# eps696/aphantasia

Hardware: AMD Instinct MI355X
Metric: optimization steps/sec @1280x720 ViT-B/32 samples=200 (higher is better)
Workload: dtype f16 (MFMA operands, fp32 accumulate; fp32 residual stream / LayerNorm / softmax statistics / synth / sampler / loss / Adam)

## Files before the change

### aphantasia_amd/_ffi.py

```python
import ctypes
import os
from ctypes import POINTER, c_char_p, c_float, c_int, c_size_t, c_void_p

import torch

HERE = os.path.dirname(os.path.abspath(__file__))
LIB_PATH = os.path.join(HERE, 'libaphantasia_hip.so')

APH_OUT_NCHW_RAW, APH_OUT_NCHW_NORM, APH_OUT_PATCH_F16, APH_GRAD_PATCH_F16, APH_OUT_PATCH_F16_HILO, APH_OUT_PATCH_F32 = 0, 1, 2, 3, 4, 5
APH_AUG_STRIDE = 16
SIM_TYPES = {'cossim': 0, 'cos': 0, None: 0, 'mix': 1, 'ang': 2, 'dot': 3}


class SampleGeom(ctypes.Structure):
    _fields_ = [(n, c_int) for n in ('H', 'W', 'Hp', 'Wp', 'py0', 'px0', 'S', 'size', 'patch')]


_PROTOTYPES = {
    'aph_version': (c_int, []),
    'aph_last_error': (c_char_p, []),
    'aph_synth_plan_create': (c_int, [c_int, c_int, c_int, POINTER(c_void_p)]),
    'aph_synth_plan_destroy': (c_int, [c_void_p]),
    'aph_synth_fft_fwd': (c_int, [c_void_p, c_void_p, c_void_p, c_void_p, c_float, POINTER(c_float), c_int, c_void_p, c_void_p, c_void_p]),
    'aph_synth_fft_bwd': (c_int, [c_void_p, c_void_p, c_float, c_void_p, c_void_p, c_void_p, c_float, POINTER(c_float), c_int, c_void_p, c_void_p]),
    'aph_irfft2': (c_int, [c_void_p, c_void_p, c_void_p, c_void_p]),
    'aph_rfft2': (c_int, [c_void_p, c_void_p, c_void_p, c_void_p]),
    'aph_synth_spatial_fwd': (c_int, [c_void_p, c_void_p, c_float, c_float, POINTER(c_float), c_int, c_void_p, c_void_p]),
    'aph_synth_spatial_bwd': (c_int, [c_void_p, c_void_p, c_float, c_void_p, c_void_p, c_float, c_float, POINTER(c_float), c_int, c_void_p, c_void_p]),
    'aph_synth_stats': (c_int, [c_void_p, c_void_p, c_void_p]),
    'aph_synth_set_stats': (c_int, [c_void_p, c_void_p, c_void_p]),
    'aph_synth_plan_describe': (c_int, [c_void_p, POINTER(c_int)]),
    'aph_idwt_coarse_levels': (c_int, [POINTER(c_int), POINTER(c_int), c_int, c_int]),
    'aph_rgb_priors_ws_bytes': (c_size_t, []),
    'aph_rgb_sharp': (c_int, [c_void_p, c_int, c_int, c_float, c_void_p, c_void_p, c_void_p, c_void_p]),
    'aph_rgb_priors': (c_int, [c_void_p, c_int, c_int, c_float, c_float, c_float, c_void_p, c_void_p, c_void_p, c_void_p]),
    'aph_cppn_param_count': (c_size_t, [c_int, c_int, c_int]),
    'aph_cppn_ws_bytes': (c_size_t, [c_int, c_int, c_int, c_int, c_int]),
    'aph_cppn_fwd': (c_int, [c_void_p, c_int, c_int, c_int, c_void_p, c_void_p, c_int, c_int, c_void_p, c_void_p, c_void_p]),
    'aph_cppn_bwd': (c_int, [c_void_p, c_int, c_int, c_int, c_void_p, c_void_p, c_int, c_int, c_void_p, c_float, c_void_p, c_void_p, c_void_p, c_void_p]),
    'aph_idwt_level_fwd': (c_int, [c_void_p, c_int, c_int, c_void_p, c_int, c_int, c_int, c_void_p, c_void_p, c_int, c_float, c_void_p, c_void_p]),
    'aph_idwt_fwd': (c_int, [c_void_p, c_void_p, c_void_p, c_void_p, c_void_p, c_int, c_int, c_void_p, c_void_p, c_int, c_void_p, c_void_p]),
    'aph_idwt_bwd': (c_int, [c_void_p, c_void_p, c_void_p, c_void_p, c_int, c_int, c_void_p, c_void_p, c_int, c_void_p, c_void_p, c_void_p, c_void_p]),
    'aph_idwt_level_bwd': (c_int, [c_void_p, c_int, c_int, c_int, c_void_p, c_void_p, c_int, c_float, c_void_p, c_int, c_int, c_void_p, c_void_p]),
    'aph_sample_ws_bytes': (c_size_t, [POINTER(SampleGeom), c_int]),
    'aph_sample_fwd': (c_int, [POINTER(SampleGeom), c_void_p, c_void_p, c_void_p, c_void_p, c_void_p, c_int, c_void_p]),
    'aph_sample_bwd': (c_int, [POINTER(SampleGeom), c_void_p, c_float, c_void_p, c_void_p, c_void_p, c_void_p, c_int, c_void_p]),
    'aph_triangle_blur': (c_int, [c_void_p, c_int, c_int, c_int, c_int, c_float, c_float, c_void_p, c_void_p]),
    'aph_resize_bicubic': (c_int, [c_void_p, c_int, c_int, c_int, c_void_p, c_int, c_int, c_void_p]),
    'aph_flip_w': (c_int, [c_void_p, c_void_p, c_int, c_int, c_int, c_void_p, c_void_p]),
    'aph_grid_warp': (c_int, [c_void_p, c_void_p, c_int, c_int, c_int, c_float, c_float, c_float, c_float, c_float, c_void_p, c_void_p, c_void_p]),
    'aph_attn_test': (c_int, [c_void_p, c_void_p, c_void_p, c_void_p, c_void_p, c_void_p, c_int, c_int, c_int, c_int, c_void_p]),
    'aph_attn_f32_test': (c_int, [c_void_p, c_void_p, c_void_p, c_void_p, c_void_p, c_void_p, c_int, c_int, c_int, c_int, c_void_p]),
    'aph_frame_affine': (c_int, [c_void_p, c_int, c_int, c_int, POINTER(c_float), c_void_p, c_void_p]),
    'aph_patchify_f16': (c_int, [c_void_p, c_int, c_int, c_int, c_void_p, c_void_p]),
    'aph_patchify_f16_hilo': (c_int, [c_void_p, c_int, c_int, c_int, c_void_p, c_void_p]),
    'aph_patchify_f32': (c_int, [c_void_p, c_int, c_int, c_int, c_void_p, c_void_p]),
    'aph_unpatchify_f32': (c_int, [c_void_p, c_int, c_int, c_int, c_float, c_void_p, c_void_p]),
    'aph_vit_create': (c_int, [c_int, c_int, c_int, c_int, c_int, c_int, c_int, POINTER(c_void_p)]),
    'aph_vit_destroy': (c_int, [c_void_p]),
    'aph_vit_workspace_bytes': (c_size_t, [c_void_p]),
    'aph_vit_set_weight': (c_int, [c_void_p, c_char_p, c_void_p, c_size_t]),
    'aph_vit_forward': (c_int, [c_void_p, c_void_p, c_int, c_void_p, c_void_p]),
    'aph_vit_forward_hilo': (c_int, [c_void_p, c_void_p, c_int, c_void_p, c_void_p]),
    'aph_vit_enable_hilo': (c_int, [c_void_p]),
    'aph_vit_enable_f32': (c_int, [c_void_p]),
    'aph_vit_forward_f32': (c_int, [c_void_p, c_void_p, c_int, c_void_p, c_void_p]),
    'aph_vit_backward_f32': (c_int, [c_void_p, c_void_p, c_int, c_void_p, c_float, c_void_p]),
    'aph_vit_backward': (c_int, [c_void_p, c_void_p, c_int, c_void_p, c_float, c_void_p]),
    'aph_vit_backward_h': (c_int, [c_void_p, c_void_p, c_int, c_void_p, c_float, c_void_p]),
    'aph_vit_profile': (c_int, [c_void_p, c_int]),
    'aph_vit_profile_read': (c_int, [c_void_p, c_void_p, c_void_p, c_void_p]),
    'aph_gemm_set_mfma32': (c_int, [c_int]),
    'aph_vit_set_fuse_ln': (c_int, [c_int]),
    'aph_crop_adjoint_set_gather': (c_int, [c_int]),
    'aph_crop_adjoint_set_shape': (c_int, [c_int, c_int, c_int, c_int, c_int]),
    'aph_vit_set_grad_stream_f16': (c_int, [c_int]),
    'aph_gemm_set_ws_min_tiles': (c_int, [c_int]),
    'aph_gemm_set_ws_pgroup': (c_int, [c_int]),
    'aph_gemm_set_rs': (c_int, [c_int]),
    'aph_mfma_rate': (c_int, [c_int, c_int, c_void_p, c_void_p, c_void_p]),
    'aph_gemm_rs_probe': (c_int, [c_void_p, c_void_p, c_int, c_int, c_int, c_void_p, c_int, c_void_p, c_void_p]),
    'aph_gemm_ws_probe': (c_int, [c_void_p, c_void_p, c_int, c_int, c_int, c_void_p, c_void_p, c_void_p, c_int, c_void_p, c_void_p]),
    'aph_gemm_f32_test': (c_int, [c_void_p, c_int, c_int, c_void_p, c_int, c_int, c_int, c_int, c_void_p, c_int, c_void_p, c_void_p, c_int, c_void_p, c_size_t, c_void_p]),
    'aph_gemm_f16': (c_int, [c_void_p, c_void_p, c_int, c_int, c_int, c_void_p, c_void_p]),
    'aph_gemm_f16_ld': (c_int, [c_void_p, c_int, c_void_p, c_int, c_int, c_int, c_int, c_void_p, c_int, c_void_p]),
    'aph_gemm_f16_epi_test': (c_int, [c_void_p, c_int, c_void_p, c_int, c_int, c_int, c_int, c_void_p, c_int, c_void_p, c_void_p, c_void_p, c_float, c_int,
                                      c_int, c_int, c_int, c_void_p, c_size_t, c_int, c_void_p]),
    'aph_ln_test': (c_int, [c_int, c_int, c_int, c_int, c_int, c_int, c_int, c_void_p, c_void_p, c_void_p, c_void_p, c_void_p, c_void_p, c_void_p,
                            c_void_p, c_void_p, c_void_p, c_void_p, c_void_p, c_void_p, c_void_p]),
    'aph_sim_loss': (c_int, [c_void_p, c_int, c_int, c_void_p, c_void_p, POINTER(c_float), c_int, c_int, c_int, c_int, c_int, c_float, c_float, c_void_p, c_void_p, c_void_p, c_void_p]),
    'aph_axpy_f32': (c_int, [c_void_p, c_void_p, c_float, c_size_t, c_void_p]),
    'aph_rgb_to_u8': (c_int, [c_void_p, c_int, c_int, c_float, c_void_p, c_void_p]),
    'aph_linear_head': (c_int, [c_void_p, c_int, c_int, c_void_p, c_float, c_float, c_float, c_float, c_void_p, c_void_p, c_void_p]),
    'aph_comm_unique_id': (c_int, [c_void_p]),
    'aph_comm_init': (c_int, [c_int, c_int, c_void_p, POINTER(c_void_p)]),
    'aph_allreduce_f32': (c_int, [c_void_p, c_void_p, c_size_t, c_void_p]),
    'aph_comm_ranks': (c_int, [c_void_p, POINTER(c_int)]),
    'aph_comm_destroy': (c_int, [c_void_p]),
    'aph_adam_step': (c_int, [c_void_p, c_void_p, c_void_p, c_void_p, c_void_p, c_void_p, c_int, c_size_t, c_void_p]),
    'aph_adam_step_guarded': (c_int, [c_void_p, c_void_p, c_void_p, c_void_p, c_void_p, c_void_p, c_int, c_size_t, c_void_p, c_void_p]),
}

EXPORTS = tuple(_PROTOTYPES)

class Library:

    def __init__(self, path):
        if not os.path.isfile(path):
            raise RuntimeError(
                "aphantasia_amd: HIP library not found at %s -- build it with "
                "`python -c 'import __graft_entry__ as g; g.build()'` (hipcc, gfx950). "
                "There is no CPU fallback." % path)
        self.path = path
        self.cdll = ctypes.CDLL(path)
        for name, (res, args) in _PROTOTYPES.items():
            fn = getattr(self.cdll, name)
            fn.restype = res
            fn.argtypes = args

    def last_error(self):
        return (self.cdll.aph_last_error() or b'').decode(errors='replace')

    def call(self, name, *args):
        rc = getattr(self.cdll, name)(*args)
        if rc < 0:
            raise RuntimeError('%s failed (%d): %s' % (name, rc, self.last_error()))
        return rc


_lib = None


def lib():
    global _lib
    if _lib is None:
        import torch
        if torch.cuda.is_available():
            torch.cuda.init()
            torch.empty(1, device='cuda')
        _lib = Library(LIB_PATH)
    return _lib


def ptr(t):
    return c_void_p(t.data_ptr()) if t is not None else c_void_p(0)


def floats(seq):
    if seq is None:
        return None
    arr = (c_float * len(seq))(*[float(v) for v in seq])
    return arr
```

### aphantasia_amd/csrc/vit_gemm_ws.h

```cpp
#pragma once
#include "vit_gemm.h"

namespace aph {

template <int BM_, int NPROD_, int NSTAGE_, int WG_PER_CU_, int BIAS_MAX_, int FORCE_WAVES_ = 0>
struct GemmWSCfg {
  static constexpr int BM = BM_, BN = 128, WM = BM / 64, WN = 2, NCONS = WM * WN, NPROD = NPROD_, NWAVE = NCONS + NPROD, NTHREAD = NWAVE * 64;
  static constexpr int NSTAGE = NSTAGE_, WG_PER_CU = WG_PER_CU_;
  static constexpr int STAGE = (BM + BN) * GEMM_BK;
  static constexpr int SMEM = NSTAGE * STAGE * 2;
  static constexpr int BIAS_MAX = BIAS_MAX_;
  static constexpr int SMEM_TOTAL = SMEM + BIAS_MAX * 4;
  static constexpr int QA = BM / 8, QB = BN / 8;
  static constexpr int QPW = (QA + QB) / NPROD;
  static constexpr int QAW = QA / NPROD;
  static constexpr int MIN_WAVES_PER_SIMD = FORCE_WAVES_ ? FORCE_WAVES_ : (WG_PER_CU * NWAVE + 3) / 4;
  static_assert(QA % NPROD == 0 && QB % NPROD == 0 && (NSTAGE - 1) * QPW <= 63, "the DMA in flight must fit the vmcnt range");
  static_assert(WG_PER_CU * SMEM_TOTAL <= 160 * 1024 && NSTAGE >= 2 && NSTAGE <= 3, "LDS budget / ring depth");
};
using GemmWS = GemmWSCfg<256, 2, 3, 1, 4096>;

__host__ __device__ __forceinline__ int gemm_ws_brow(int v) {
  const int vv = v & 63, nt = vv >> 4, i = vv & 15;
  return (v & ~63) + (i << 2) + nt;
}

__device__ __forceinline__ half4 pack_h4(float a, float b, float c, float d) { return half4{(half_t)a, (half_t)b, (half_t)c, (half_t)d}; }

#define APH_WS_ROWS(r, m4, M) for (int r = 0; r < 4; ++r) if ((m4) + r < (M))
__device__ __forceinline__ void ws_tile(const EpiF16& e, int m4, int M, int n4, f32x4 (&v)[4], const float* lb) {
  f32x4 b = {0.f, 0.f, 0.f, 0.f};
  if (e.bias) b = *reinterpret_cast<const f32x4*>(lb + n4);
#pragma unroll
  APH_WS_ROWS(r, m4, M)
    *reinterpret_cast<half4*>(e.out + (size_t)(m4 + r) * e.ldo + n4) = pack_h4(v[0][r] + b[0], v[1][r] + b[1], v[2][r] + b[2], v[3][r] + b[3]);
}
__device__ __forceinline__ void ws_tile(const EpiF16Scale& e, int m4, int M, int n4, f32x4 (&v)[4], const float*) {
#pragma unroll
  APH_WS_ROWS(r, m4, M)
    *reinterpret_cast<half4*>(e.out + (size_t)(m4 + r) * e.ldo + n4) = pack_h4(v[0][r] * e.scale, v[1][r] * e.scale, v[2][r] * e.scale, v[3][r] * e.scale);
}
__device__ __forceinline__ void ws_tile(const EpiF32& e, int m4, int M, int n4, f32x4 (&v)[4], const float*) {
#pragma unroll
  APH_WS_ROWS(r, m4, M) st4(e.out + (size_t)(m4 + r) * e.ldo + n4, f32x4{v[0][r], v[1][r], v[2][r], v[3][r]} * e.scale);
}
__device__ __forceinline__ void ws_tile(const EpiNoStore& e, int m4, int M, int n4, f32x4 (&v)[4], const float*) {
  const f32x4 t = v[0] + v[1] + v[2] + v[3];
  if (m4 < M && t[0] + t[1] + t[2] + t[3] == 1.2345678e33f) st4(e.out + (size_t)m4 * e.ldo + n4, t);
}
__device__ __forceinline__ void ws_tile(const EpiResidual& e, int m4, int M, int n4, f32x4 (&v)[4], const float*) {
#pragma unroll
  APH_WS_ROWS(r, m4, M) st4(e.out + (size_t)(m4 + r) * e.ldo + n4, f32x4{v[0][r], v[1][r], v[2][r], v[3][r]});
}
__device__ __forceinline__ void ws_tile(const EpiPatchEmbed& e, int m4, int M, int n4, f32x4 (&v)[4], const float*) {
#pragma unroll
  APH_WS_ROWS(r, m4, M) {
    const int m = m4 + r, s = m / e.P, p = m - s * e.P;
    st4(e.x0 + ((size_t)s * e.T + 1 + p) * e.D + n4, f32x4{v[0][r], v[1][r], v[2][r], v[3][r]} + ld4(e.pos + (size_t)(1 + p) * e.D + n4));
  }
}
__device__ __forceinline__ void ws_tile(const EpiGelu& e, int m4, int M, int n4, f32x4 (&v)[4], const float* lb) {
  const f32x4 b = *reinterpret_cast<const f32x4*>(lb + n4);
#pragma unroll
  for (int r = 0; r < 4; ++r) {
    f32x4 gl, dg;
    quick_gelu4(f32x4{v[0][r] + b[0], v[1][r] + b[1], v[2][r] + b[2], v[3][r] + b[3]}, gl, dg);
    if (m4 + r < M) {
      *reinterpret_cast<half4*>(e.g + (size_t)(m4 + r) * e.ldo + n4) = pack_h4(gl[0], gl[1], gl[2], gl[3]);
      *reinterpret_cast<half4*>(e.dg + (size_t)(m4 + r) * e.ldo + n4) = pack_h4(dg[0], dg[1], dg[2], dg[3]);
    }
  }
}
__device__ __forceinline__ void ws_tile(const EpiGeluBwd& e, int m4, int M, int n4, f32x4 (&v)[4], const half4 (&d)[4]) {
#pragma unroll
  APH_WS_ROWS(r, m4, M)
    *reinterpret_cast<half4*>(e.out + (size_t)(m4 + r) * e.ldo + n4) =
        pack_h4(v[0][r] * (float)d[r][0], v[1][r] * (float)d[r][1], v[2][r] * (float)d[r][2], v[3][r] * (float)d[r][3]);
}
#undef APH_WS_ROWS
template <class E>
__device__ __forceinline__ void ws_tiles(const E& e, int m4, int M, int n4, f32x4 (&acc)[4][4], const float* lb) {
#pragma unroll
  for (int mt = 0; mt < 4; ++mt) ws_tile(e, m4 + mt * 16, M, n4, acc[mt], lb);
}
__device__ __forceinline__ void ws_tiles(const EpiGeluBwd& e, int m4, int M, int n4, f32x4 (&acc)[4][4], const float*) {
  half4 d[4][4];
#pragma unroll
  for (int mt = 0; mt < 4; ++mt)
#pragma unroll
    for (int r = 0; r < 4; ++r) {
      const int m = m4 + mt * 16 + r;
      d[mt][r] = *reinterpret_cast<const half4*>(e.dg + (size_t)(m < M ? m : M - 1) * e.ldo + n4);
    }
#pragma unroll
  for (int mt = 0; mt < 4; ++mt) ws_tile(e, m4 + mt * 16, M, n4, acc[mt], d[mt]);
}
template <class E>
__device__ __forceinline__ void ws_init(const E&, int, int, int, f32x4 (&v)[4], const float*) {
#pragma unroll
  for (int j = 0; j < 4; ++j) v[j] = f32x4{0.f, 0.f, 0.f, 0.f};
}
__device__ __forceinline__ void ws_init(const EpiResidual& e, int m4, int M, int n4, f32x4 (&v)[4], const float*) {
  const f32x4 b = ld4(e.bias + n4);
#pragma unroll
  for (int r = 0; r < 4; ++r) {
    const int m = m4 + r < M ? m4 + r : M - 1;
    const f32x4 x = ld4(e.res + (size_t)m * e.ldo + n4) + b;
    v[0][r] = x[0]; v[1][r] = x[1]; v[2][r] = x[2]; v[3][r] = x[3];
  }
}
__device__ __forceinline__ const float* ws_bias(const EpiF16& e) { return e.bias; }
__device__ __forceinline__ const float* ws_bias(const EpiResidual& e) { return e.bias; }
__device__ __forceinline__ const float* ws_bias(const EpiGelu& e) { return e.bias; }
template <class E> __device__ __forceinline__ const float* ws_bias(const E&) { return nullptr; }

__device__ __forceinline__ unsigned long long ws_realtime() {
#ifdef APH_EMU
  return 0ull;
#else
  return __builtin_amdgcn_s_memrealtime();
#endif
}
__device__ __forceinline__ unsigned long long ws_clock() {
#ifdef APH_EMU
  return 0ull;
#else
  return __builtin_amdgcn_s_memtime();
#endif
}

template <int AHEAD_UNIT>
__device__ __forceinline__ void ws_wait_barrier(int ahead) {
  if (ahead <= 0) wait_vm_barrier<0>();
  else if (ahead == 1) wait_vm_barrier<AHEAD_UNIT>();
  else wait_vm_barrier<(2 * AHEAD_UNIT <= 63 ? 2 * AHEAD_UNIT : 63)>();
}

template <class C, class Epi>
__global__ __launch_bounds__(C::NTHREAD, C::MIN_WAVES_PER_SIMD) void gemm_ws_kernel(const half_t* __restrict__ A, int lda, const half_t* __restrict__ Bt,
                                                                  int ldb, int M, int N, int K, Epi epi, int ntiles, int pgroup, unsigned long long* __restrict__ trace,
                                                                  int ntn_short, int nk_short) {
  using F = GemmBig;
  APH_DYN_SMEM(smem);
  half_t* lds = reinterpret_cast<half_t*>(smem);
  const int tid = threadIdx.x, lane = tid & 63, wave = wave_uniform(tid >> 6);
  const int nk = K / GEMM_BK, ntn = N / C::BN, ntm = ntiles / ntn, ntn_long = ntn - ntn_short;
  int pos, pos_end, tile_step, lstart, sstart, nlong;
  {
    const int nwg = gridDim.x, b = blockIdx.x, G = nwg < 8 ? nwg : 8, xcd = b % G;
    auto share = [&](int n, int& start, int& count) {
      const int q = n / G, r = n - q * G;
      start = xcd < r ? xcd * (q + 1) : r * (q + 1) + (xcd - r) * q;
      count = q + (xcd < r ? 1 : 0);
    };
    int nshort;
    share(ntm * ntn_long, lstart, nlong);
    share(ntm * ntn_short, sstart, nshort);
    pos_end = nlong + nshort;
    tile_step = (nwg - xcd + G - 1) / G;
    pos = b / G;
  }
  if (pos >= pos_end) return;
  if (trace && tid == 0) trace[((size_t)blockIdx.x * 16 + 15) * 4 + 3] = ws_realtime();
  int U = 0;
  for (int q = pos; q < pos_end; q += tile_step) U += q < nlong ? nk : nk_short;
  auto coords = [&](int q, int& tm, int& tn) -> int {
    const bool lng = q < nlong;
    const int t = lng ? lstart + q : sstart + (q - nlong), cols = lng ? ntn_long : ntn_short;
    const int per = pgroup * cols, g = t / per, rem = t - g * per;
    const int left = ntm - g * pgroup, rg = left < pgroup ? left : pgroup;
    tn = rem / rg;
    tm = g * pgroup + (rem - tn * rg);
    if (!lng) tn += ntn_long;
    return lng ? nk : nk_short;
  };
  float* lbias = reinterpret_cast<float*>(smem + C::SMEM);
  if (const float* gb = ws_bias(epi)) {
    for (int i = tid * 4; i < N; i += C::NTHREAD * 4) *reinterpret_cast<f32x4*>(lbias + i) = ld4(gb + i);
    wait_lgkm0();
  }

  if (wave >= C::NCONS) {
    const int p = wave - C::NCONS, lrow = lane >> 3, pc = lane & 7;
    unsigned off[C::QPW];
    const char* Ab = reinterpret_cast<const char*>(A);
    const char* Bb = reinterpret_cast<const char*>(Bt);
    int nk_it = nk;
    auto setup = [&](int t) {
      int tm, tn;
      nk_it = coords(t, tm, tn);
      const int n0 = tn * C::BN, m0 = tm * C::BM;
#pragma unroll
      for (int i = 0; i < C::QPW; ++i) {
        if (i < C::QAW) {
          const int row = (i * C::NPROD + p) * 8 + lrow;
          int am = m0 + row; am = am < M ? am : M - 1;
          off[i] = ((unsigned)am * (unsigned)lda + ((pc ^ ((row >> 1) & 7)) << 3)) * 2u;
        } else {
          const int v = ((i - C::QAW) * C::NPROD + p) * 8 + lrow;
          off[i] = ((unsigned)(n0 + gemm_ws_brow(v)) * (unsigned)ldb + ((pc ^ ((v >> 1) & 7)) << 3)) * 2u;
        }
      }
    };
    auto issue = [&](int kt, int stage) {
      half_t* As = lds + stage * C::STAGE;
      half_t* Bs = As + C::BM * GEMM_BK;
      const char* ak = Ab + (size_t)kt * (GEMM_BK * 2);
      const char* bk = Bb + (size_t)kt * (GEMM_BK * 2);
#pragma unroll
      for (int i = 0; i < C::QPW; ++i) {
        if (i < C::QAW) glds16(ak + off[i], As + (i * C::NPROD + p) * 8 * GEMM_BK);
        else glds16(bk + off[i], Bs + ((i - C::QAW) * C::NPROD + p) * 8 * GEMM_BK);
      }
    };
    int it = pos, ikt = 0, ist = 0, issued = 0;
    setup(it);
    auto issue_next = [&]() {
      issue(ikt, ist);
      ist = ist == C::NSTAGE - 1 ? 0 : ist + 1;
      ++issued;
      if (++ikt == nk_it) {
        ikt = 0;
        it += tile_step;
        if (issued < U) setup(it);
      }
    };
    const int pre = U < C::NSTAGE - 1 ? U : C::NSTAGE - 1;
    for (int i = 0; i < pre; ++i) issue_next();
    ws_wait_barrier<C::QPW>(pre - 1);
    if (U > C::NSTAGE - 1) issue_next();
    for (int u = 0; u + 1 < U; ++u) {
      const int rem = U - u - 2;
      ws_wait_barrier<C::QPW>(rem < C::NSTAGE - 2 ? rem : C::NSTAGE - 2);
      if (u + C::NSTAGE < U) issue_next();
    }
    return;
  }

  const int wm = wave / C::WN, wn = wave - wm * C::WN;
  f32x4 acc[F::TM][F::TN];
  const int frow = lane & 15, arow = wm * 64 + frow, brow = wn * 64 + frow, fchunk = lane >> 4;
  GemmFrags<F> f0, f1;
  int kt = 0, st = 0, nk_c = nk, ti = 0;
  auto init_tile = [&](int t) {
    int tm, tn;
    nk_c = coords(t, tm, tn);
    const int m4 = tm * C::BM + wm * 64 + 4 * (lane >> 4), n4 = tn * C::BN + wn * 64 + 4 * (lane & 15);
#pragma unroll
    for (int mt = 0; mt < F::TM; ++mt) ws_init(epi, m4 + mt * 16, M, n4, acc[mt], lbias);
  };
  auto mma = [&](const GemmFrags<F>& f) {
#pragma unroll
    for (int mt = 0; mt < F::TM; ++mt)
#pragma unroll
      for (int nt = 0; nt < F::TN; ++nt) acc[mt][nt] = mfma_16x16x32_f16(f.a[mt], f.b[nt], acc[mt][nt]);
  };
  init_tile(pos);
  wait_vm_barrier<63>();
  gemm_load_frags<F>(f0, lds, lds + C::BM * GEMM_BK, arow, brow, fchunk);
  for (int u = 0; u < U; ++u) {
    const half_t* As = lds + st * C::STAGE;
    st = st == C::NSTAGE - 1 ? 0 : st + 1;
    gemm_load_frags<F>(f1, As, As + C::BM * GEMM_BK, arow, brow, 4 + fchunk);
    mma(f0);
    if (u + 1 < U) {
      wait_lgkm0();
      wait_vm_barrier<63>();
      const half_t* An = lds + st * C::STAGE;
      gemm_load_frags<F>(f0, An, An + C::BM * GEMM_BK, arow, brow, fchunk);
    }
    mma(f1);
    if (trace && kt == 0 && tid == 0 && ti < 14) trace[((size_t)blockIdx.x * 16 + ti) * 4 + 0] = ws_clock();
    if (++kt == nk_c) {
      if (trace && tid == 0 && ti < 14) trace[((size_t)blockIdx.x * 16 + ti) * 4 + 1] = ws_clock();
      int tm, tn;
      coords(pos, tm, tn);
      const int m4 = tm * C::BM + wm * 64 + 4 * (lane >> 4), n4 = tn * C::BN + wn * 64 + 4 * (lane & 15);
      ws_tiles(epi, m4, M, n4, acc, lbias);
      if (trace && tid == 0 && ti < 14) trace[((size_t)blockIdx.x * 16 + ti) * 4 + 2] = ws_clock();
      kt = 0;
      ++ti;
      pos += tile_step;
      if (u + 1 < U) init_tile(pos);
    }
  }
  if (trace && tid == 0) trace[((size_t)blockIdx.x * 16 + 14) * 4 + 3] = ws_realtime();
}

inline int& gemm_ws_pgroup_override() {
  static int v = 0;
  return v;
}
inline int gemm_ws_panel_group(int ntn, int ntm) {
  int g = gemm_ws_pgroup_override();
  if (g <= 0) g = ntn >= 12 ? 4 : 1;
  return g < ntm ? g : (ntm > 0 ? ntm : 1);
}

template <class C, class Epi>
inline void launch_gemm_ws_cfg(const half_t* A, int lda, const half_t* Bt, int ldb, int M, int N, int K, Epi epi, hipStream_t st,
                               unsigned long long* trace, int n_short = 0, int k_short = 0) {
  const int ntiles = (N / C::BN) * ((M + C::BM - 1) / C::BM);
  const int cus = gemm_persistent_wgs();
  const int wgs = cus > (1 << 20) ? cus : cus * C::WG_PER_CU;
  APH_ALLOW_SMEM((gemm_ws_kernel<C, Epi>), C::SMEM_TOTAL);
  APH_LAUNCH((gemm_ws_kernel<C, Epi>), dim3(ntiles < wgs ? ntiles : wgs), dim3(C::NTHREAD), C::SMEM_TOTAL, st, A, lda, Bt, ldb, M, N, K, epi, ntiles,
             gemm_ws_panel_group(N / C::BN, (M + C::BM - 1) / C::BM), trace, n_short / C::BN, k_short / GEMM_BK);
}
template <class Epi>
inline void launch_gemm_ws(const half_t* A, int lda, const half_t* Bt, int ldb, int M, int N, int K, Epi epi, hipStream_t st,
                           unsigned long long* trace, int n_short, int k_short) {
  launch_gemm_ws_cfg<GemmWS>(A, lda, Bt, ldb, M, N, K, epi, st, trace, n_short, k_short);
}

}
```

Baseline: 167.1.

## Overlap tile epilogue with first k-step MFMAs of next persistent tile

In the warp-specialized persistent GEMM, when a tile finishes and more work remains, the epilogue of the finished tile is interleaved row-block by row-block with the first k-step MFMAs of the next tile, instead of running the whole epilogue before the main loop resumes. Scheduling fences keep the compiler from reordering the epilogue stores and MFMAs. This is meant to hide epilogue latency between tiles, but it adds register pressure and more complex control flow. Residual and GELU-backward epilogues are excluded, and a turnover toggle (default on) is exposed through the FFI.

```diff
diff --git a/aphantasia_amd/_ffi.py b/aphantasia_amd/_ffi.py
--- a/aphantasia_amd/_ffi.py
+++ b/aphantasia_amd/_ffi.py
@@ -77,6 +77,7 @@
     'aph_vit_set_grad_stream_f16': (c_int, [c_int]),
     'aph_gemm_set_ws_min_tiles': (c_int, [c_int]),
     'aph_gemm_set_ws_pgroup': (c_int, [c_int]),
+    'aph_gemm_set_ws_turnover': (c_int, [c_int]),
     'aph_gemm_set_rs': (c_int, [c_int]),
     'aph_mfma_rate': (c_int, [c_int, c_int, c_void_p, c_void_p, c_void_p]),
     'aph_gemm_rs_probe': (c_int, [c_void_p, c_void_p, c_int, c_int, c_int, c_void_p, c_int, c_void_p, c_void_p]),
diff --git a/aphantasia_amd/csrc/vit_gemm_ws.h b/aphantasia_amd/csrc/vit_gemm_ws.h
--- a/aphantasia_amd/csrc/vit_gemm_ws.h
+++ b/aphantasia_amd/csrc/vit_gemm_ws.h
@@ -95,6 +95,14 @@
 #pragma unroll
   for (int mt = 0; mt < 4; ++mt) ws_tile(e, m4 + mt * 16, M, n4, acc[mt], d[mt]);
 }
+template <class E> struct WsPipelined { static constexpr bool value = true; };
+template <> struct WsPipelined<EpiResidual> { static constexpr bool value = false; };
+template <> struct WsPipelined<EpiGeluBwd> { static constexpr bool value = false; };
+__device__ __forceinline__ void ws_sched_fence() {
+#ifndef APH_EMU
+  __builtin_amdgcn_sched_barrier(0);
+#endif
+}
 template <class E>
 __device__ __forceinline__ void ws_init(const E&, int, int, int, f32x4 (&v)[4], const float*) {
 #pragma unroll
@@ -136,7 +144,7 @@
   else wait_vm_barrier<(2 * AHEAD_UNIT <= 63 ? 2 * AHEAD_UNIT : 63)>();
 }
 
-template <class C, class Epi>
+template <class C, class Epi, bool PIPE>
 __global__ __launch_bounds__(C::NTHREAD, C::MIN_WAVES_PER_SIMD) void gemm_ws_kernel(const half_t* __restrict__ A, int lda, const half_t* __restrict__ Bt,
                                                                   int ldb, int M, int N, int K, Epi epi, int ntiles, int pgroup, unsigned long long* __restrict__ trace,
                                                                   int ntn_short, int nk_short) {
@@ -272,16 +280,57 @@
     mma(f1);
     if (trace && kt == 0 && tid == 0 && ti < 14) trace[((size_t)blockIdx.x * 16 + ti) * 4 + 0] = ws_clock();
     if (++kt == nk_c) {
-      if (trace && tid == 0 && ti < 14) trace[((size_t)blockIdx.x * 16 + ti) * 4 + 1] = ws_clock();
-      int tm, tn;
-      coords(pos, tm, tn);
-      const int m4 = tm * C::BM + wm * 64 + 4 * (lane >> 4), n4 = tn * C::BN + wn * 64 + 4 * (lane & 15);
-      ws_tiles(epi, m4, M, n4, acc, lbias);
-      if (trace && tid == 0 && ti < 14) trace[((size_t)blockIdx.x * 16 + ti) * 4 + 2] = ws_clock();
-      kt = 0;
-      ++ti;
-      pos += tile_step;
-      if (u + 1 < U) init_tile(pos);
+      for (;;) {
+        if (trace && tid == 0 && ti < 14) trace[((size_t)blockIdx.x * 16 + ti) * 4 + 1] = ws_clock();
+        int tm, tn;
+        coords(pos, tm, tn);
+        const int m4 = tm * C::BM + wm * 64 + 4 * (lane >> 4), n4 = tn * C::BN + wn * 64 + 4 * (lane & 15);
+        bool turn = false;
+        if constexpr (PIPE) turn = u + 1 < U;
+        if (!turn) {
+          ws_tiles(epi, m4, M, n4, acc, lbias);
+          if (trace && tid == 0 && ti < 14) trace[((size_t)blockIdx.x * 16 + ti) * 4 + 2] = ws_clock();
+          kt = 0;
+          ++ti;
+          pos += tile_step;
+          if (u + 1 < U) init_tile(pos);
+          break;
+        }
+        if constexpr (PIPE) {
+          pos += tile_step;
+          nk_c = coords(pos, tm, tn);
+          const int m4n = tm * C::BM + wm * 64 + 4 * (lane >> 4), n4n = tn * C::BN + wn * 64 + 4 * (lane & 15);
+          const half_t* A1 = lds + st * C::STAGE;
+          st = st == C::NSTAGE - 1 ? 0 : st + 1;
+          gemm_load_frags<F>(f1, A1, A1 + C::BM * GEMM_BK, arow, brow, 4 + fchunk);
+          ++u;
+  #pragma unroll
+          for (int mt = 0; mt < F::TM; ++mt) {
+            ws_tile(epi, m4 + mt * 16, M, n4, acc[mt], lbias);
+            ws_init(epi, m4n + mt * 16, M, n4n, acc[mt], lbias);
+            ws_sched_fence();
+  #pragma unroll
+            for (int nt = 0; nt < F::TN; ++nt) acc[mt][nt] = mfma_16x16x32_f16(f0.a[mt], f0.b[nt], acc[mt][nt]);
+            if (mt == 0) {
+              wait_lgkm0();
+              if (u + 1 < U) wait_vm_barrier<63>();
+            }
+            if (mt == F::TM - 1 && u + 1 < U) {
+              ws_sched_fence();
+              const half_t* An = lds + st * C::STAGE;
+              gemm_load_frags<F>(f0, An, An + C::BM * GEMM_BK, arow, brow, fchunk);
+            }
+  #pragma unroll
+            for (int nt = 0; nt < F::TN; ++nt) acc[mt][nt] = mfma_16x16x32_f16(f1.a[mt], f1.b[nt], acc[mt][nt]);
+            ws_sched_fence();
+          }
+          if (trace && tid == 0 && ti < 14) trace[((size_t)blockIdx.x * 16 + ti) * 4 + 2] = ws_clock();
+          ++ti;
+          if (trace && tid == 0 && ti < 14) trace[((size_t)blockIdx.x * 16 + ti) * 4 + 0] = ws_clock();
+          kt = 1;
+          if (kt != nk_c) break;
+        }
+      }
     }
   }
   if (trace && tid == 0) trace[((size_t)blockIdx.x * 16 + 14) * 4 + 3] = ws_realtime();
@@ -297,15 +346,28 @@
   return g < ntm ? g : (ntm > 0 ? ntm : 1);
 }
 
+inline int& gemm_ws_turnover() {
+  static int v = 1;
+  return v;
+}
+
+template <class C, class Epi, bool PIPE>
+inline void launch_gemm_ws_pipe(const half_t* A, int lda, const half_t* Bt, int ldb, int M, int N, int K, Epi epi, hipStream_t st,
+                                unsigned long long* trace, int n_short, int k_short) {
+  const int ntiles = (N / C::BN) * ((M + C::BM - 1) / C::BM);
+  const int cus = gemm_persistent_wgs();
+  const int wgs = cus > (1 << 20) ? cus : cus * C::WG_PER_CU;
+  APH_ALLOW_SMEM((gemm_ws_kernel<C, Epi, PIPE>), C::SMEM_TOTAL);
+  APH_LAUNCH((gemm_ws_kernel<C, Epi, PIPE>), dim3(ntiles < wgs ? ntiles : wgs), dim3(C::NTHREAD), C::SMEM_TOTAL, st, A, lda, Bt, ldb, M, N, K, epi, ntiles,
+             gemm_ws_panel_group(N / C::BN, (M + C::BM - 1) / C::BM), trace, n_short / C::BN, k_short / GEMM_BK);
+}
 template <class C, class Epi>
 inline void launch_gemm_ws_cfg(const half_t* A, int lda, const half_t* Bt, int ldb, int M, int N, int K, Epi epi, hipStream_t st,
                                unsigned long long* trace, int n_short = 0, int k_short = 0) {
-  const int ntiles = (N / C::BN) * ((M + C::BM - 1) / C::BM);
-  const int cus = gemm_persistent_wgs();
-  const int wgs = cus > (1 << 20) ? cus : cus * C::WG_PER_CU;
-  APH_ALLOW_SMEM((gemm_ws_kernel<C, Epi>), C::SMEM_TOTAL);
-  APH_LAUNCH((gemm_ws_kernel<C, Epi>), dim3(ntiles < wgs ? ntiles : wgs), dim3(C::NTHREAD), C::SMEM_TOTAL, st, A, lda, Bt, ldb, M, N, K, epi, ntiles,
-             gemm_ws_panel_group(N / C::BN, (M + C::BM - 1) / C::BM), trace, n_short / C::BN, k_short / GEMM_BK);
+  if constexpr (WsPipelined<Epi>::value) {
+    if (gemm_ws_turnover()) return launch_gemm_ws_pipe<C, Epi, true>(A, lda, Bt, ldb, M, N, K, epi, st, trace, n_short, k_short);
+  }
+  launch_gemm_ws_pipe<C, Epi, false>(A, lda, Bt, ldb, M, N, K, epi, st, trace, n_short, k_short);
 }
 template <class Epi>
 inline void launch_gemm_ws(const half_t* A, int lda, const half_t* Bt, int ldb, int M, int N, int K, Epi epi, hipStream_t st,
```

Result: no change. 168.5, median of 6 (+0.9%).
